# ohinder/OnePhase.jl

Measured on AMD Instinct MI355X. Metric: KKT factor+solve/sec (fp64) at n+m~1e5, nnz~2e6, higher is better.
Workload: dtype f64

## Files before the change

onephase.jl_amd/csrc/asan_driver.cpp:

```cpp
#include <cstdio>
#include <cstdlib>
#include <random>
#include <set>
#include <vector>

#include "numeric.h"
#include "pivots.h"
#include "symbolic.h"

using namespace okkt;

static void csc_lower(int n, const std::set<std::pair<int, int>>& e, std::vector<int64_t>& cp, std::vector<int64_t>& ri) {
  std::vector<std::vector<int>> cols(n);
  for (auto& p : e) cols[std::min(p.first, p.second)].push_back(std::max(p.first, p.second));
  cp.assign(n + 1, 0); ri.clear();
  for (int j = 0; j < n; ++j) { ri.push_back(j); for (int r : cols[j]) if (r != j) ri.push_back(r); cp[j + 1] = (int64_t)ri.size(); }
}

static int run(const char* name, int n, const std::set<std::pair<int, int>>& e, int ordering) {
  std::vector<int64_t> cp, ri;
  csc_lower(n, e, cp, ri);
  SymbolicOptions o;
  o.ordering = ordering;
  Symbolic S;
  const std::string err = analyze_pattern(n, cp.data(), ri.data(), 0, o, nullptr, S);
  if (!err.empty()) { fprintf(stderr, "%s (ordering %d): %s\n", name, ordering, err.c_str()); return 1; }
  std::vector<DfFront> fronts;
  for (int s = 0; s < (int)S.sn_col0.size() - 1 && fronts.size() < 3; ++s) {
    const int k = S.sn_col0[s + 1] - S.sn_col0[s], f = (int)(S.row_ptr[s + 1] - S.row_ptr[s]);
    if (f > 128) fronts.push_back({s, f, k});
  }
  size_t ntask = 0;
  if (!fronts.empty()) {
    std::vector<DfTask> q;
    double model = 0;
    df_build_queue(fronts, 64, 4, 1, true, true, q, &model, true);
    ntask = q.size();
    df_build_queue(fronts, 96, 2, 2, false, false, q, &model, false);
  }
  std::vector<int64_t> fpos(S.nsuper + 1, 0);
  for (int s = 0; s < S.nsuper; ++s)
    fpos[s + 1] = fpos[s] + (S.row_ptr[s + 1] - S.row_ptr[s]) * (int64_t)(S.sn_col0[s + 1] - S.sn_col0[s]);
  for (int skip : {-1, S.nsuper - 1}) {
    PvPlan P;
    const std::string pe = pivot_build_items(S, fpos, 128, skip, P);
    if (!pe.empty()) { fprintf(stderr, "%s (ordering %d): %s\n", name, ordering, pe.c_str()); return 1; }
    std::vector<int> seen(n, 0), next_row(n, -1);
    int64_t entries = 0;
    bool ok = true;
    for (const PvSmall& q : P.small) {
      ok = ok && q.f <= 128 && q.k <= q.f && q.L >= 0 && q.L + (int64_t)q.f * q.k <= fpos[S.nsuper];
      for (int lc = 0; lc < q.k; ++lc) { ++seen[q.col0 + lc]; entries += q.f - lc - 1; }
    }
    std::vector<int> part_owner(P.nparts, -1);
    for (const PvBig& q : P.big) {
      const int s = S.col2sn[q.out], f = (int)(S.row_ptr[s + 1] - S.row_ptr[s]), lc = q.out - S.sn_col0[s];
      ok = ok && f > 128 && q.col == fpos[s] + (int64_t)lc * f && q.rows == S.row_ptr[s] && q.r0 <= q.r1 && q.r1 <= f && q.r1 - q.r0 <= kPvChunkRows;
      ok = ok && q.r0 == (next_row[q.out] < 0 ? lc + 1 : next_row[q.out]);
      next_row[q.out] = q.r1;
      entries += q.r1 - q.r0;
      if (q.part < 0) ++seen[q.out];
      else { ok = ok && q.part < P.nparts && part_owner[q.part] < 0; if (ok) part_owner[q.part] = q.out; }
    }
    for (const PvMerge& q : P.merge) {
      ++seen[q.out];
      ok = ok && q.nparts > 1 && q.part0 >= 0 && q.part0 + q.nparts <= P.nparts;
      for (int c = 0; ok && c < q.nparts; ++c) ok = part_owner[q.part0 + c] == q.out;
    }
    const int ncov = skip < 0 ? n : S.sn_col0[skip];
    for (int c = 0; c < n; ++c) {
      ok = ok && seen[c] == (c < ncov ? 1 : 0);
      if (c < ncov && next_row[c] >= 0) { const int s = S.col2sn[c]; ok = ok && next_row[c] == (int)(S.row_ptr[s + 1] - S.row_ptr[s]); }
    }
    ok = ok && entries == P.entries && P.ncols == ncov;
    if (!ok) { fprintf(stderr, "%s (ordering %d): the pivot-report items do not tile the factor (skip %d)\n", name, ordering, skip); return 1; }
  }
  printf("%-12s ordering %d: n %d nnz(L) %lld supernodes %zu, %zu dataflow tasks\n", name, ordering, n, (long long)S.nnzL, S.sn_col0.size() - 1, ntask);
  return 0;
}

int main() {
  int bad = 0;
  std::mt19937 rng(5);
  {
    const int n = 3000;
    std::set<std::pair<int, int>> e;
    for (int i = 0; i < n; ++i) for (int d = 1; d <= 3; ++d) if (i + d < n) e.insert({i, i + d});
    for (int i = 0; i < n; i += 2) e.insert({i, n - 1});
    for (int o : {0, 3, 4}) bad += run("banded", n, e, o);
  }
  {
    const int g = 14, n = g * g * g;
    std::set<std::pair<int, int>> e;
    auto id = [&](int x, int y, int z) { return (x * g + y) * g + z; };
    for (int x = 0; x < g; ++x) for (int y = 0; y < g; ++y) for (int z = 0; z < g; ++z) {
      if (x + 1 < g) e.insert({id(x, y, z), id(x + 1, y, z)});
      if (y + 1 < g) e.insert({id(x, y, z), id(x, y + 1, z)});
      if (z + 1 < g) e.insert({id(x, y, z), id(x, y, z + 1)});
    }
    for (int o : {0, 3, 4, 5}) bad += run("grid", n, e, o);
  }
  {
    const int n = 12000;
    std::set<std::pair<int, int>> e;
    for (int i = 0; i < n; ++i) for (int d = 1; d <= 12; d += 3) if (i + d < n) e.insert({i, i + d});
    for (int t = 0; t < n / 4; ++t) { const int a = (int)(rng() % n), b = (int)(rng() % n); if (a != b) e.insert({a, b}); }
    for (int o : {0, 5}) bad += run("small-world", n, e, o);
  }
  {
    const int n = 24000;
    std::set<std::pair<int, int>> e;
    for (int i = 0; i < n; ++i) for (int d = 1; d <= 12; d += 3) if (i + d < n) e.insert({i, i + d});
    for (int t = 0; t < n / 4; ++t) { const int a = (int)(rng() % n), b = (int)(rng() % n); if (a != b) e.insert({a, b}); }
    bad += run("small-world-24k", n, e, 5);
  }
  {
    const int n = 600;
    std::set<std::pair<int, int>> e;
    for (int i = 0; i + 1 < n; ++i) { e.insert({i, n - 1}); e.insert({i, i + 1}); }
    for (int o : {0, 1, 3}) bad += run("arrow", n, e, o);
  }
  {
    const int n = 2300;
    std::set<std::pair<int, int>> e;
    for (int i = 1; i < n; ++i) e.insert({0, i});
    bad += run("full-column", n, e, 1);
  }
  if (bad) { fprintf(stderr, "%d case(s) failed\n", bad); return 1; }
  printf("asan driver: all cases clean\n");
  return 0;
}
```

onephase.jl_amd/csrc/numeric.h:

```cpp
#pragma once
#include <hip/hip_runtime.h>

#include <cstdint>
#include <string>
#include <vector>

#include "symbolic.h"

namespace okkt {

struct EaRec { int64_t src; int64_t rel; int rc; int jj; int64_t cut; };
static_assert(sizeof(EaRec) == 32, "two 16-byte loads per record");

struct DevPlan {
  int n = 0, nsuper = 0;
  int has_dup = 0;
  int* sn_col0 = nullptr;
  int64_t* row_ptr = nullptr;
  int* rows = nullptr;
  int64_t* front_pos = nullptr;
  int64_t* cb_shift = nullptr;
  int64_t* child_ptr = nullptr;
  int* children = nullptr;
  int64_t* rel_ptr = nullptr;
  int* rel = nullptr;
  int64_t* cv_pos = nullptr;
  int64_t* aent_ptr = nullptr;
  int64_t* aent_src = nullptr;
  int64_t* aent_dst = nullptr;
  int* perm = nullptr;
  int* sched = nullptr;
  int* task_lo = nullptr;
  int* unit_parent = nullptr;
  double* arena = nullptr;
  const double* vals = nullptr;
  double* dvals = nullptr;
  double* diagadd = nullptr;
  double* xwork = nullptr;
  double* zwork = nullptr;
  double* cv = nullptr;
  double* wbuf = nullptr;
  int64_t* wbuf_pos = nullptr;
  int64_t* bigcol_base = nullptr;
  int64_t* ea_ptr = nullptr;
  int* ea_child = nullptr;
  int* ea_jj = nullptr;
  int64_t* ea_pos = nullptr;
  int* ea_rc = nullptr;
  int64_t* ea_src = nullptr;
  int64_t* ea_rel = nullptr;
  int64_t* ea_cut = nullptr;
  const struct EaRec* ea_rec = nullptr;
  int* cutv = nullptr;
  int64_t* acol_lo = nullptr;
  double* xinv = nullptr;
  double* xtmp = nullptr;
  int64_t* xinv_pos = nullptr;
  double* ypart = nullptr;
  int64_t* ypart_pos = nullptr;
  int solve_mid = 0;
  double* ythin = nullptr;
  int64_t* ythin_pos = nullptr;
  int* ssched = nullptr;
  unsigned long long* sver = nullptr;
  int64_t* sver_pos = nullptr;
  int64_t xw_stride = 0, cv_stride = 0;
  double* invl = nullptr;
  int64_t* invl_pos = nullptr;
  int* sn_owner = nullptr;
  int* col_owner = nullptr;
  int* top_cols = nullptr;
  int* bnd = nullptr;
  int64_t* bnd_cb = nullptr;
  int64_t* bnd_cv = nullptr;
  unsigned long long* counters = nullptr;
  long long want_pos = -1, want_neg = -1;
  double* zero_page = nullptr;
  int df_early_pub = 1;
  int* df_state = nullptr;
  int64_t* df_state_pos = nullptr;
};

enum { kDfD = 0, kDfT = 1, kDfU = 2, kDfTU = 3, kDfTA = 4, kDfTL = 5 };
struct DfTask { int front; int type_nq; int ij; int q0; };
struct DfFront { int s, f, k; };
void df_build_queue(const std::vector<DfFront>& fronts, int workers, int group, int rows_per_task, bool fuse_d, bool split_tu, std::vector<DfTask>& out, double* model_us,
                    bool fuse_tl = false, bool multi_rows = true);
// ... 78 lines not shown
  int flow_levels = 0, flow_off = 0, flow_cnt = 0, flow_maxf = 0, flow_maxk = 0;
  int* flow_flags = nullptr;
  int flow_epoch = 0;
  int dataflow = 1;
  int df_group = 4;
  int df_fuse_d = 1;
  int df_split_tu = 1;
  std::vector<int64_t> front_pos_host;
  int64_t arena_doubles = 0;
  int64_t cb_region_doubles = 0;
  int release_cb = 1;
  int df_fuse_tl = 1;
  int df_rows = 1;
  int df_workers = 256;
  DfTask* df_tasks = nullptr;
  int* df_heads = nullptr;
  int n_df_heads = 0;
  int64_t df_state_ints = 0;
  int diag2 = 1;
  int lookahead = 1;
  int sb_tail_rows = 4000;
  int la_min_tiles = 600;
  std::vector<hipEvent_t> la_events;
  size_t la_used = 0;
  double* vals_owned = nullptr;
  int64_t nnz_in = 0;
  bool profile = false;
  std::vector<hipEvent_t> prof_events;
  size_t prof_used = 0;
  std::vector<double> prof_flops;
  std::vector<std::pair<int, int>> big_fk;
  std::vector<int> sched_host;
  std::vector<int> sn_f, sn_k;
  int schur_sn = -1;
  int64_t schur_gcb = 0;
  int* schur_list = nullptr;
};

std::string numeric_setup(const Symbolic& S, const SymbolicOptions& opts, hipStream_t stream, Numeric& N);
void numeric_release(Numeric& N);

std::string numeric_factor_enqueue(Numeric& N, const double* d_vals, double tol, int which = 0, bool reset_counters = true);
std::string solve_fwd_enqueue(Numeric& N, int which, int R);
std::string solve_bwd_enqueue(Numeric& N, int which, int R);
std::string solve_setup(const Symbolic& S, Numeric& N);
std::string solve_invert_enqueue(Numeric& N, hipStream_t st, const SolveLevel& L, int b_lo, int b_hi);
void solve_permute_in(const Numeric& N, const double* d_rhs, int64_t stride, int nr, int R, const double* d_scale = nullptr);
void solve_permute_out(const Numeric& N, double* d_sol, int64_t stride, int nr, int R, bool accumulate, const double* d_scale = nullptr);
std::string numeric_dist_pack(Numeric& N, int what, int unpack, double* d_buf);
std::string numeric_dist_x(Numeric& N, int mode, double* d_buf);
void numeric_sum_counts_device(Numeric& N, long long* d_out4);
std::string schur_condense_enqueue(Numeric& N, double* d_r2, int nr, int R);
std::string schur_expand_enqueue(Numeric& N, const double* d_x2, int nr, int R);
std::string schur_gather_enqueue(Numeric& N, double* d_r2, int nr, int R);
std::string schur_put_enqueue(Numeric& N, const double* d_x2, int nr, int R);
void schur_export_enqueue(Numeric& N, double* d_S, int64_t ld);
std::string numeric_solve_enqueue(Numeric& N, int R);
void launch_set_shift(const Numeric& N, double delta, int64_t nshift);
std::string df_setup(Numeric& N);
const char* df_build_flags();
std::string df_launch(Numeric& N, const DevPlan& P, const Segment& g, hipStream_t st, double tol);

}
```

onephase.jl_amd/csrc/numeric.hip:

```cpp
#include "numeric.h"
#include "front_device.h"
#include <map>

#include <algorithm>
#include <cmath>
#include <cstdio>
#include <cstdlib>

namespace okkt {


#define OKKT_HIP_TRY(expr)                                                         \
  do {                                                                             \
    hipError_t e__ = (expr);                                                       \
    if (e__ != hipSuccess)                                                         \
      return std::string(#expr) + ": " + hipGetErrorString(e__);                   \
  } while (0)

__global__ void k_fold_counts(DevPlan P) {
  const int c = threadIdx.x;
  if (c >= 4) return;
  unsigned long long sum = 0;
  for (int q = 1; q < kCountSlots; ++q) {
    unsigned long long* w = P.counters + (size_t)q * kCountStride + c;
// ... 305 lines not shown
    }
    int d[NB4];
    double v[NB4];
#pragma unroll
    for (int u = 0; u < NB4; ++u) {
      const int ii = min(lo[u] + lane, rc[u] - 1);
      d[u] = P.rel[rel[u] + ii] - r0;
      v[u] = P.arena[src[u] + ii];
    }
#pragma unroll
    for (int u = 0; u < NB4; ++u) {
      if (q + u < q1) {
        if (lo[u] + lane < hi[u]) base[d[u]] += v[u];
        const int* rl = P.rel + rel[u];
        const double* Ccol = P.arena + src[u];
        int ii = lo[u] + 64 + lane;
        for (; ii + 64 * (kAsmUnroll - 1) < hi[u]; ii += 64 * kAsmUnroll) {
          int dd[kAsmUnroll];
          double vv[kAsmUnroll], oo[kAsmUnroll];
#pragma unroll
          for (int w = 0; w < kAsmUnroll; ++w) dd[w] = rl[ii + 64 * w] - r0;
#pragma unroll
          for (int w = 0; w < kAsmUnroll; ++w) { vv[w] = Ccol[ii + 64 * w]; oo[w] = base[dd[w]]; }
#pragma unroll
          for (int w = 0; w < kAsmUnroll; ++w) base[dd[w]] = oo[w] + vv[w];
        }
        for (; ii < hi[u]; ii += 64) base[rl[ii] - r0] += Ccol[ii];
        __threadfence_block();
      }
    }
  }
  double* col = P.arena + P.front_pos[s] + (size_t)pc * f + r0 + cb_off(P, s, pc, k);
  for (int i = lane; i < n; i += 64) col[i] = base[i];
}






__global__ __launch_bounds__(256) void k_big_diag(DevPlan P, const int* __restrict__ list, int step, int NB, double tol, int dbg_stop) {
  extern __shared__ __attribute__((aligned(16))) double sm[];
  const int tid = threadIdx.x, lane = tid & 63;
  const int wave = __builtin_amdgcn_readfirstlane(tid >> 6);
  const int l15 = lane & 15, l4 = lane >> 4;
  const int s = list[blockIdx.x];
  if (stop_requested_wg(P)) return;
  const int col0 = P.sn_col0[s];
  const int k = P.sn_col0[s + 1] - col0;
  const int f = (int)(P.row_ptr[s + 1] - P.row_ptr[s]);
  const int j0 = step * NB;
  if (j0 >= k) return;
  const int nb = min(NB, k - j0);
  double* Praw = sm;
  double* Lp = Praw + kMW * kPLD;
  double* Wp = Lp + kMW * kPLD;
  double* Ld = Wp + kMW * kPLD;
  double* Xs = Ld + 4 * 32 * kXld;
  double* F = P.arena + P.front_pos[s];

  int ti_s[9], tj_s[9];
#pragma unroll
  for (int q = 0; q < 9; ++q) {
    const int t = 4 * q + wave;
    const int tj = (t >= 8) + (t >= 15) + (t >= 21) + (t >= 26) + (t >= 30) + (t >= 33) + (t >= 35);
    const int start = tj * 8 - tj * (tj - 1) / 2;
// ... 665 lines not shown
        }
      }
      if (wlevel > 0) { wregion[wlevel_seq & 1] = std::max(wregion[wlevel_seq & 1], wlevel); ++wlevel_seq; }
    }
  };
  build(N.levels, parted ? N.part_id : 0);
  if (parted && N.part_id == 0) build(N.levels_top, -1); else N.levels_top.clear();
  if (!(e = upload(N, sched, &d.sched)).empty()) return e;
  if (!(e = upload(N, task_lo, &d.task_lo)).empty()) return e;
  N.flow_levels = N.flow_off = N.flow_cnt = N.flow_maxf = N.flow_maxk = 0;
  if (N.flow && (!parted || parted_tasks)) {
    int nl = 0;
    while (nl < (int)N.levels.size() && N.levels[nl].seg[3].cnt == 0) ++nl;
    if (nl >= 2) {
      N.flow_levels = nl;
      N.flow_off = N.levels[0].seg[0].off;
      for (int l = 0; l < nl; ++l)
        for (int c = 0; c < 3; ++c) { N.flow_cnt += N.levels[l].seg[c].cnt; if (N.levels[l].seg[c].cnt) { N.flow_maxf = std::max(N.flow_maxf, N.levels[l].seg[c].maxf); N.flow_maxk = std::max(N.flow_maxk, N.levels[l].seg[c].maxk); } }
      if (N.flow_cnt == 0) N.flow_levels = 0;
    }
  }
  {
    std::vector<int> unit_parent(ns, -1);
    for (int s2 = 0; s2 < ns; ++s2) {
      if (unit_root[s2] != s2 || S.sn_parent[s2] < 0) continue;
      const int up = unit_root[S.sn_parent[s2]];
      if (up == N.schur_sn) continue;
      if (ulevel[up] < N.flow_levels && (!parted || S.sn_owner[up] == S.sn_owner[s2])) unit_parent[s2] = up;
    }
    if (!(e = upload(N, unit_parent, &d.unit_parent)).empty()) return e;
  }
  if (getenv("OKKT_DEBUG_FRONTS")) fprintf(stderr, "okkt: %d levels of units (%d levels of fronts), %lld tasks of small fronts, longest %d\n", nulev, S.nlevels, (long long)N.n_tasks, N.max_task_len);
  N.release_cb = getenv("OKKT_RELEASE_CB") ? atoi(getenv("OKKT_RELEASE_CB")) : 1;
  if (parted) N.release_cb = 0;
  std::vector<int64_t> fpos(ns + 1, 0), cbshift(ns, 0);
  if (!N.release_cb) {
    for (int s2 = 0; s2 <= ns; ++s2) fpos[s2] = S.front_pos[s2];
    N.arena_doubles = S.arena_doubles;
    N.cb_region_doubles = 0;
  } else {
    for (int s2 = 0; s2 < ns; ++s2) {
      const int64_t f = S.row_ptr[s2 + 1] - S.row_ptr[s2], k = S.sn_col0[s2 + 1] - S.sn_col0[s2];
      fpos[s2 + 1] = fpos[s2] + ((f * k + 1) & ~(int64_t)1);
    }
    const int64_t panels = fpos[ns];
    auto epoch_of = [&](int s2) { const int l = ulevel[unit_root[s2]]; return l < N.flow_levels ? 0 : l - std::max(N.flow_levels, 1) + 1; };
    const int nep = std::max(1, nulev - std::max(N.flow_levels, 1) + 1) + 1;
    std::vector<std::vector<int>> born(nep), dies(nep);
    for (int s2 = 0; s2 < ns; ++s2) {
      const int64_t f = S.row_ptr[s2 + 1] - S.row_ptr[s2], k = S.sn_col0[s2 + 1] - S.sn_col0[s2];
      if (f == k) continue;
      const int p2 = S.sn_parent[s2];
      born[epoch_of(s2)].push_back(s2);
      dies[p2 >= 0 && p2 != N.schur_sn ? epoch_of(p2) : nep - 1].push_back(s2);
    }
    std::map<int64_t, int64_t> freeb;
    int64_t top = 0;
    std::vector<int64_t> cbo(ns, -1), cbsz(ns, 0);
    auto release = [&](int64_t off, int64_t sz) {
      auto it = freeb.emplace(off, sz).first;
      auto nx = std::next(it);
      if (nx != freeb.end() && it->first + it->second == nx->first) { it->second += nx->second; freeb.erase(nx); }
      if (it != freeb.begin()) { auto pv = std::prev(it); if (pv->first + pv->second == it->first) { pv->second += it->second; freeb.erase(it); it = pv; } }
      if (it->first + it->second == top) { top = it->first; freeb.erase(it); }
    };
    for (int ep = 0; ep < nep; ++ep) {
// ... 115 lines not shown
      for (int64_t q = S.rel_ptr[c]; q < S.rel_ptr[c + 1]; ++q) {
        const int64_t slot = fill[bigcol_base[p] + S.rel[q]]++;
        ea_child[slot] = c;
        ea_jj[slot] = (int)(q - S.rel_ptr[c]);
        ea_pos[slot] = S.cv_pos[c] + (q - S.rel_ptr[c]);
        {
          const int64_t kc = S.sn_col0[c + 1] - S.sn_col0[c], fc = S.row_ptr[c + 1] - S.row_ptr[c];
          ea_rc[slot] = (int)(fc - kc);
          ea_rel[slot] = S.rel_ptr[c];
          ea_cut[slot] = cut_pos[c];
          ea_src[slot] = fpos[c] + cbshift[c] + (kc + ea_jj[slot]) * fc + kc;
        }
      }
    }
    if (!(e = upload(N, bigcol_base, &d.bigcol_base)).empty()) return e;
    if (!(e = upload(N, invl_pos, &d.invl_pos)).empty()) return e;
    if (!(e = upload(N, ea_ptr, &d.ea_ptr)).empty()) return e;
    if (!(e = upload(N, ea_child, &d.ea_child)).empty()) return e;
    if (!(e = upload(N, ea_jj, &d.ea_jj)).empty()) return e;
    if (!(e = upload(N, ea_pos, &d.ea_pos)).empty()) return e;
    if (!(e = upload(N, ea_rc, &d.ea_rc)).empty()) return e;
    if (!(e = upload(N, ea_src, &d.ea_src)).empty()) return e;
    if (!(e = upload(N, ea_rel, &d.ea_rel)).empty()) return e;
    if (!(e = upload(N, ea_cut, &d.ea_cut)).empty()) return e;
    {
      std::vector<EaRec> recs(ea_src.size());
      for (size_t t = 0; t < recs.size(); ++t) recs[t] = EaRec{ea_src[t], ea_rel[t], ea_rc[t], ea_jj[t], ea_cut[t]};
      EaRec* dr = nullptr;
      if (!(e = upload(N, recs, &dr)).empty()) return e;
      d.ea_rec = dr;
    }
    if (!(e = upload(N, cutv, &d.cutv)).empty()) return e;
    if (!(e = upload(N, acol_lo, &d.acol_lo)).empty()) return e;
    if (N.schur_sn >= 0) {
      N.schur_gcb = bigcol_base[N.schur_sn];
      if (!(e = upload(N, std::vector<int>{N.schur_sn}, &N.schur_list)).empty()) return e;
    }
    if (!(e = dalloc(N, (size_t)invl_total, &d.invl, true)).empty()) return e;
  }
  if (!(e = dalloc(N, (size_t)N.arena_doubles + 512 + (size_t)S.max_front * 2, &d.arena, false)).empty()) return e;
  if (!(e = dalloc(N, (size_t)S.n, &d.dvals, true)).empty()) return e;
  if (!(e = dalloc(N, (size_t)S.n, &d.diagadd, true)).empty()) return e;
  d.xw_stride = S.n;
  d.cv_stride = S.sum_r;
  if (!(e = dalloc(N, (size_t)S.n * kMaxRhs, &d.xwork, true)).empty()) return e;
  if (!(e = dalloc(N, (size_t)S.n * kMaxRhs, &d.zwork, true)).empty()) return e;
  if (!(e = dalloc(N, (size_t)S.sum_r * kMaxRhs, &d.cv, true)).empty()) return e;
  if (!(e = dalloc(N, (size_t)wtotal + 512, &d.wbuf, true)).empty()) return e;
  if (!(e = dalloc(N, (size_t)kCountSlots * kCountStride, &d.counters, true)).empty()) return e;
  if (!(e = dalloc(N, (size_t)512, &d.zero_page, true)).empty()) return e;
  if (!(e = dalloc(N, (size_t)S.nnz_in, &N.vals_owned, false)).empty()) return e;
  {
    double* raw = nullptr;
    if (!(e = dalloc(N, (size_t)ns / 2 + 8, &raw, true)).empty()) return e;
    N.chain_flags = (int*)raw;
    N.chain_epoch = 0;
    raw = nullptr;
    if (!(e = dalloc(N, (size_t)3 * ns / 2 + 8, &raw, true)).empty()) return e;
    N.flow_flags = (int*)raw;
    N.flow_epoch = 0;
  }
  if (!(e = solve_setup(S, N)).empty()) return e;
  if (!(e = df_setup(N)).empty()) return e;
  const int big_lds = 160 * 1024 - 64;
  OKKT_HIP_TRY(hipFuncSetAttribute((const void*)k_front_small<256>, hipFuncAttributeMaxDynamicSharedMemorySize, big_lds));
  OKKT_HIP_TRY(hipFuncSetAttribute((const void*)k_front_small<256, true>, hipFuncAttributeMaxDynamicSharedMemorySize, big_lds));
// ... 64 lines not shown
std::string numeric_factor_enqueue(Numeric& N, const double* d_vals, double tol, int which, bool reset_counters) {
  DevPlan P = N.d;
  P.vals = d_vals;
  hipStream_t st = N.stream;
  {
    const size_t na = reset_counters ? (size_t)kCountSlots * kCountStride * (sizeof(unsigned long long) / sizeof(unsigned)) : 0;
    const size_t nb = (reset_counters && N.solve_counters) ? (size_t)N.d.nsuper : 0;
    const size_t nc = (N.dataflow && P.df_state) ? (size_t)N.df_state_ints + (size_t)N.n_df_heads * kDfHeadStride : 0;
    if (na + nb + nc) {
      const unsigned grid = (unsigned)std::min<size_t>(2048, (na + nb + nc + 1023) / 1024);
      hipLaunchKernelGGL(k_zero_words, dim3(grid), dim3(256), 0, st, (unsigned*)P.counters, na, (unsigned*)N.solve_counters, nb, (unsigned*)P.df_state, nc);
    }
  }
  if (N.early_check && N.early_device && which == 0 && N.levels_top.empty() && reset_counters) { P.want_pos = N.early_n; P.want_neg = N.early_m; }
  N.la_used = 0;
  if (which == 0) {
    for (size_t l = 0; l < N.inv_level_pending.size(); ++l)
      if (N.inv_level_pending[l] && N.inv_level_events[l]) OKKT_HIP_TRY(hipStreamWaitEvent(st, N.inv_level_events[l], 0));
    if (N.inv_wait && N.inv_event) OKKT_HIP_TRY(hipStreamWaitEvent(st, N.inv_event, 0));
  }
  if (which == 0) std::fill(N.inv_level_pending.begin(), N.inv_level_pending.end(), 0);
  if (which == 0) N.inv_wait = false;
  bool inv_on_aux = false;
  N.early_exited = false;
  std::string e;
  {
    const LaneStreams ss{N.stream, N.stream_masked, N.stream_panel, N.stream_aux};
    e = factor_sched(N, P, which == 0 ? N.levels : N.levels_top, which == 0 ? N.slevels : N.slevels_top, ss, tol,
                     which == 0 && N.levels_top.empty(), inv_on_aux);
    if (!e.empty()) return e;
  }
  if (which == 0 && N.schur_sn >= 0) {
    const int f = N.sn_f[N.schur_sn];
    if (f > 2048) hipLaunchKernelGGL(k_big_assemble_chunked, dim3((f + 3) / 4, 1, (f + kAsmChunk - 1) / kAsmChunk), dim3(256), 0, st, P, N.schur_list);
    else {
      const int lcol = std::max(256, (f + 63) / 64 * 64);
      hipLaunchKernelGGL(k_big_assemble<true>, dim3((f + 3) / 4, 1), dim3(256), (size_t)4 * lcol * sizeof(double), st, P, N.schur_list, lcol);
    }
  }
  const bool per_level = which == 0 && N.levels_top.empty() && !N.inv_level_pending.empty();
  if (inv_on_aux && !per_level) {
    if (!N.inv_event) OKKT_HIP_TRY(hipEventCreateWithFlags(&N.inv_event, hipEventDisableTiming));
    OKKT_HIP_TRY(hipEventRecord(N.inv_event, N.inv_stream ? N.inv_stream : N.stream_aux));
    N.inv_wait = true;
  }
  OKKT_HIP_TRY(hipGetLastError());
  return "";
}

static std::string factor_sched(Numeric& N, DevPlan P, const std::vector<LevelSchedule>& levels, const std::vector<SolveLevel>& slevels,
                                const LaneStreams& ss, double tol, bool in_loop_check, bool& inv_on_aux, size_t l_begin, size_t l_end) {
  const hipStream_t cur = ss.main;
  const int NB = N.nb;
  static const int dbg_syrk = getenv("OKKT_DEBUG_SYRK") ? atoi(getenv("OKKT_DEBUG_SYRK")) : 0;
  static const int split_min_rows = getenv("OKKT_SPLIT_MIN_ROWS") ? atoi(getenv("OKKT_SPLIT_MIN_ROWS")) : 5000;
  static const int dbg_stop = getenv("OKKT_DEBUG_DIAG_STOP") ? atoi(getenv("OKKT_DEBUG_DIAG_STOP")) : 0;
  static const int fuse_max_fronts = getenv("OKKT_FUSE_MAX_FRONTS") ? atoi(getenv("OKKT_FUSE_MAX_FRONTS")) : 8;
  for (size_t l = l_begin; l < std::min(l_end, levels.size()); ++l) {
    const LevelSchedule& L = levels[l];
    if (N.early_check && in_loop_check && (int)l == N.early_level) {
      unsigned long long cnt[6] = {0, 0, 0, 0, 0, 0};
      std::string ec = numeric_read_counts(N, cur, cnt);
      if (!ec.empty()) return ec;
      if (cnt[4] != 0 || cnt[3] > 0 || cnt[2] > 0 || cnt[1] > (unsigned long long)N.early_m || cnt[0] > (unsigned long long)N.early_n) {
        N.early_exited = true;
        return "";
      }
// ... 30 lines not shown
        const int rows_after = g.maxf - (stepA + GS) * NB;
        if (rows_after < N.group_one_rows) return 1;
        return (GS > N.group && rows_after < N.group_switch_rows) ? N.group : GS;
      };
      auto next_event = [&](hipEvent_t* ev) -> std::string {
        if (N.la_used >= N.la_events.size())
          for (int q = 0; q < 64; ++q) { hipEvent_t e2; OKKT_HIP_TRY(hipEventCreateWithFlags(&e2, hipEventDisableTiming)); N.la_events.push_back(e2); }
        *ev = N.la_events[N.la_used++];
        return "";
      };
      auto la_at = [&](int stepA, int gs_cur) {
        const int stepB = stepA + gs_cur;
        if (stepB >= nsteps || !N.lookahead || ss.panel == nullptr || ss.masked == nullptr) return false;
        const int remr = g.maxf - (stepB + gs_at(stepB)) * NB;
        const int Trr = remr > 0 ? (remr + 127) / 128 : 0;
        return (int64_t)Trr * (Trr + 1) / 2 * g.cnt >= N.la_min_tiles;
      };
      const bool use_df = N.dataflow && g.df_cnt > 0 && NB == 128 && dbg_syrk == 0 && dbg_stop == 0 && P.df_state != nullptr;
      const bool seg_la = !use_df && la_at(0, gs_at(0));
      hipStream_t st = cur;
      if (seg_la) {
        hipEvent_t evf;
        std::string e = next_event(&evf);
        if (!e.empty()) return e;
        OKKT_HIP_TRY(hipEventRecord(evf, ss.main));
        OKKT_HIP_TRY(hipStreamWaitEvent(ss.masked, evf, 0));
        st = ss.masked;
      }
      {
        static const int lcol_max = getenv("OKKT_ASM_LCOL") ? atoi(getenv("OKKT_ASM_LCOL")) : 2048;
        int lcol = std::min(lcol_max, std::max(256, (g.maxf + 63) / 64 * 64));
        if (lcol_max <= 0) lcol = 0;
        static const int chunked = getenv("OKKT_ASM_CHUNKED") ? atoi(getenv("OKKT_ASM_CHUNKED")) : 1;
        static const int chunk_min = getenv("OKKT_ASM_CHUNK_MIN") ? atoi(getenv("OKKT_ASM_CHUNK_MIN")) : 2048;
        if (g.maxf > chunk_min && chunked) hipLaunchKernelGGL(k_big_assemble_chunked, dim3((g.maxf + 3) / 4, g.cnt, (g.maxf + kAsmChunk - 1) / kAsmChunk), dim3(256), 0, st, P, list);
        else if (g.maxf <= 2048) hipLaunchKernelGGL(k_big_assemble<true>, dim3((g.maxf + 3) / 4, g.cnt), dim3(256), (size_t)4 * lcol * sizeof(double), st, P, list, lcol);
        else hipLaunchKernelGGL(k_big_assemble<false>, dim3((g.maxf + 3) / 4, g.cnt), dim3(256), (size_t)4 * lcol * sizeof(double), st, P, list, lcol);
      }
      auto launch_syrk = [&](hipStream_t sst, int stepA, int npan, int tstep, int head, int par, int cs, int sub = 0) -> std::string {
        const int rem = g.maxf - (head == 1 ? tstep : stepA) * NB;
        if (rem <= 0) return "";
        const int T = (rem + 127) / 128;
        const int Tr = std::max(T - cs, 0);
        int ntile = T * (T + 1) / 2;
        if (head == 1) ntile = sub == 1 ? 1 : (sub == 2 ? T - 1 : T);
        else if (head == 2) { ntile = 0; for (int c = 0; c < cs && c < T; ++c) ntile += T - c; }
        else if (head == 3) ntile = Tr * (Tr + 1) / 2;
        if (ntile == 0) return "";
        static const int small_max = getenv("OKKT_SYRK_SMALL_TILES") ? atoi(getenv("OKKT_SYRK_SMALL_TILES")) : 1500;
        const bool narrow = (head == 0 || head == 3) && dbg_syrk == 0 && (int64_t)ntile * g.cnt <= small_max;
        if (narrow) ntile = head == 0 ? T * (T + 1) : Tr * (Tr + 1);
        if (ntile <= 0) return "";
        const dim3 grid((ntile + 7) / 8 * 8, g.cnt);
        const int wofs = par * GS * NB;
        const bool prof = N.profile && (head == 0 || head == 3);
        if (prof) {
          double fl = 0;
          for (int q = 0; q < g.cnt; ++q) {
            const int s = N.sched_host[g.off + q];
            const int kk = N.sn_k[s], ff = N.sn_f[s];
            const int j0 = stepA * NB;
            if (j0 >= kk) continue;
            if (head == 1 && tstep * NB >= kk) continue;
            const double K = std::min(npan * NB, kk - j0);
            const double t0 = std::min(tstep * NB, kk);
            const double remq = ff - t0;
            const double w2 = std::min<double>(cs * 128, remq);
            const double remr = remq - w2;
// ... 271 lines not shown
```

Baseline: 56.15.

## Add staged big-front assembly kernel driven by precomputed per-chunk piece records

Precomputes on the host, per big front column and row chunk, a list of contiguous child contribution-block pieces and the range of original-matrix entries. A new kernel walks these pieces with double-buffered register loads and accumulates into an LDS column before writing it out with aligned double2 stores. It becomes the default for all big-front groups and the Schur front, replacing the older search-based chunked and whole-column assembly kernels. This is meant to cut per-item lookup and irregular-access cost during extend-add. In exchange it adds host preprocessing, device memory for the records, and launches chunked grids even for small fronts.

```diff
diff --git a/onephase.jl_amd/csrc/asan_driver.cpp b/onephase.jl_amd/csrc/asan_driver.cpp
--- a/onephase.jl_amd/csrc/asan_driver.cpp
+++ b/onephase.jl_amd/csrc/asan_driver.cpp
@@ -4,6 +4,7 @@
 #include <set>
 #include <vector>
 
+#include "asm_pieces.h"
 #include "numeric.h"
 #include "pivots.h"
 #include "symbolic.h"
@@ -15,6 +16,85 @@
   for (auto& p : e) cols[std::min(p.first, p.second)].push_back(std::max(p.first, p.second));
   cp.assign(n + 1, 0); ri.clear();
   for (int j = 0; j < n; ++j) { ri.push_back(j); for (int r : cols[j]) if (r != j) ri.push_back(r); cp[j + 1] = (int64_t)ri.size(); }
+}
+
+static bool check_asm_pieces(const Symbolic& S, int chunk) {
+  const int ns = S.nsuper;
+  std::vector<char> big(ns, 0);
+  std::vector<int64_t> cb_base(ns, 0);
+  int64_t top = 0;
+  for (int s = 0; s < ns; ++s) {
+    const int64_t f = S.row_ptr[s + 1] - S.row_ptr[s], k = S.sn_col0[s + 1] - S.sn_col0[s];
+    big[s] = f > 128;
+    cb_base[s] = top + k * f + k;
+    top += f * f + (s & 1);
+  }
+  AsmPlan A;
+  if (!asm_build_pieces(S, big, cb_base, chunk, A).empty()) return false;
+  std::vector<std::vector<int>> kids(ns);
+  for (int c = 0; c < ns; ++c) if (S.sn_parent[c] >= 0) kids[S.sn_parent[c]].push_back(c);
+  int64_t items = 0, pieces = 0;
+  for (int p = 0; p < ns; ++p) {
+    if (!big[p]) { if (A.unit_base[p] != -1) return false; continue; }
+    const int64_t f = S.row_ptr[p + 1] - S.row_ptr[p];
+    const int nchunks = (int)((f + chunk - 1) / chunk);
+    for (int64_t pc = 0; pc < f; ++pc) {
+      std::vector<int> ic, ijj, done;
+      for (int c : kids[p]) {
+        const int* rb = S.rel.data() + S.rel_ptr[c];
+        const int* re = S.rel.data() + S.rel_ptr[c + 1];
+        const int* it = std::lower_bound(rb, re, (int)pc);
+        if (it != re && *it == pc) { ic.push_back(c); ijj.push_back((int)(it - rb)); }
+      }
+      done = ijj;
+      items += (int64_t)ic.size();
+      int64_t a_next = -1;
+      for (int t = 0; t < nchunks; ++t) {
+        const AsmUnit& U = A.units[(size_t)(A.unit_base[p] + (int64_t)t * f + pc)];
+        const int64_t r0 = std::max<int64_t>(pc, (int64_t)t * chunk), r1 = std::min<int64_t>(f, (int64_t)(t + 1) * chunk);
+        if (r0 >= r1) { if (U.np != 0 || U.na != 0) return false; continue; }
+        if (U.np < 0 || U.piece0 < 0 || U.piece0 + U.np > (int64_t)A.pieces.size()) return false;
+        if (U.na < 0 || U.a0 < S.aent_ptr[p] || U.a0 + U.na > S.aent_ptr[p + 1]) return false;
+        for (int64_t e = U.a0; e < U.a0 + U.na; ++e) if (S.aent_dst[e] < pc * f + r0 || S.aent_dst[e] >= pc * f + r1) return false;
+        if (a_next >= 0 && U.a0 != a_next) return false;
+        a_next = U.a0 + U.na;
+        int q = 0;
+        for (int i = 0; i < U.np; ++i, ++pieces) {
+          const AsmPiece& R = A.pieces[(size_t)(U.piece0 + i)];
+          if (R.n <= 0) return false;
+          for (; q < (int)ic.size(); ++q) {
+            const int c = ic[q];
+            const int rc = (int)(S.rel_ptr[c + 1] - S.rel_ptr[c]);
+            if (done[q] < rc && S.rel[S.rel_ptr[c] + done[q]] < r1) break;
+          }
+          if (q == (int)ic.size()) return false;
+          const int c = ic[q];
+          const int64_t fc = S.row_ptr[c + 1] - S.row_ptr[c];
+          const int rc = (int)(S.rel_ptr[c + 1] - S.rel_ptr[c]);
+          int hi = done[q];
+          while (hi < rc && S.rel[S.rel_ptr[c] + hi] < r1) ++hi;
+          if (S.rel[S.rel_ptr[c] + done[q]] < r0) return false;
+          if (R.src != cb_base[c] + (int64_t)ijj[q] * fc + done[q] || R.rel != S.rel_ptr[c] + done[q] || R.n != hi - done[q]) return false;
+          done[q] = hi;
+          ++q;
+        }
+        for (int j = 0; j < (int)ic.size(); ++j) {
+          const int c = ic[j];
+          const int rc = (int)(S.rel_ptr[c + 1] - S.rel_ptr[c]);
+          if (done[j] < rc && S.rel[S.rel_ptr[c] + done[j]] < r1) return false;
+        }
+      }
+      for (int j = 0; j < (int)ic.size(); ++j) if (done[j] != (int)(S.rel_ptr[ic[j] + 1] - S.rel_ptr[ic[j]])) return false;
+      if (a_next >= 0) {
+        const int64_t* dst = S.aent_dst.data();
+        const int64_t lo = std::lower_bound(dst + S.aent_ptr[p], dst + S.aent_ptr[p + 1], pc * f + pc) - dst;
+        const int64_t hi = std::lower_bound(dst + S.aent_ptr[p], dst + S.aent_ptr[p + 1], (pc + 1) * f) - dst;
+        const AsmUnit& U0 = A.units[(size_t)(A.unit_base[p] + (pc / chunk) * f + pc)];
+        if (U0.a0 != lo || a_next != hi) return false;
+      }
+    }
+  }
+  return items == A.items && pieces == (int64_t)A.pieces.size();
 }
 
 static int run(const char* name, int n, const std::set<std::pair<int, int>>& e, int ordering) {
@@ -75,6 +155,8 @@
     ok = ok && entries == P.entries && P.ncols == ncov;
     if (!ok) { fprintf(stderr, "%s (ordering %d): the pivot-report items do not tile the factor (skip %d)\n", name, ordering, skip); return 1; }
   }
+  for (int chunk : {512, 1024, 48})
+    if (!check_asm_pieces(S, chunk)) { fprintf(stderr, "%s (ordering %d): the assembly pieces do not tile the extend-add items (chunk %d)\n", name, ordering, chunk); return 1; }
   printf("%-12s ordering %d: n %d nnz(L) %lld supernodes %zu, %zu dataflow tasks\n", name, ordering, n, (long long)S.nnzL, S.sn_col0.size() - 1, ntask);
   return 0;
 }
@@ -126,6 +208,17 @@
     for (int i = 1; i < n; ++i) e.insert({0, i});
     bad += run("full-column", n, e, 1);
   }
+  {
+    const int nl = 30, nsep = 2300, n = 3 * nl + nsep;
+    std::set<std::pair<int, int>> e;
+    for (int g = 0; g < 3; ++g) {
+      for (int i = 0; i < nl; ++i) for (int j = i + 1; j < nl; ++j) e.insert({g * nl + i, g * nl + j});
+      for (int i = 0; i < nl; ++i)
+        for (int r = 0; r < nsep; ++r)
+          if (g == 0 || r == 0 || (g == 1 && r % 2 == 1) || (g == 2 && (r % 3 == 2 || (r > 1020 && r < 1030)))) e.insert({g * nl + i, 3 * nl + r});
+    }
+    bad += run("three-chunks", n, e, 1);
+  }
   if (bad) { fprintf(stderr, "%d case(s) failed\n", bad); return 1; }
   printf("asan driver: all cases clean\n");
   return 0;
diff --git a/onephase.jl_amd/csrc/asm_pieces.h b/onephase.jl_amd/csrc/asm_pieces.h
--- /dev/null
+++ b/onephase.jl_amd/csrc/asm_pieces.h
@@ -0,0 +1,106 @@
+#pragma once
+#include <algorithm>
+#include <cstdint>
+#include <string>
+#include <vector>
+
+#include "symbolic.h"
+
+namespace okkt {
+
+struct alignas(16) AsmPiece { int64_t src; int rel; int n; };
+static_assert(sizeof(AsmPiece) == 16, "one 16-byte load per piece and lane");
+struct alignas(32) AsmUnit { int64_t piece0; int64_t a0; int np; int na; int pad[2]; };
+static_assert(sizeof(AsmUnit) == 32, "host and device agree on the record");
+
+struct AsmPlan {
+  std::vector<int64_t> unit_base;
+  std::vector<AsmUnit> units;
+  std::vector<AsmPiece> pieces;
+  int64_t items = 0;
+  int64_t bytes() const { return (int64_t)(unit_base.size() * sizeof(int64_t) + units.size() * sizeof(AsmUnit) + pieces.size() * sizeof(AsmPiece)); }
+};
+
+inline std::string asm_build_pieces(const Symbolic& S, const std::vector<char>& big, const std::vector<int64_t>& cb_base, int chunk, AsmPlan& A) {
+  A = AsmPlan();
+  const int ns = S.nsuper;
+  if ((int)big.size() < ns || (int)cb_base.size() < ns || chunk <= 0) return "assembly records: the inputs do not cover the supernodes";
+  if (S.rel.size() > (size_t)INT32_MAX) return "assembly records: the rel lists pass 2^31 entries";
+  A.unit_base.assign(ns, -1);
+  std::vector<int64_t> col_base(ns, -1);
+  int64_t ncols = 0, nunits = 0;
+  for (int s = 0; s < ns; ++s)
+    if (big[s]) {
+      const int64_t f = S.row_ptr[s + 1] - S.row_ptr[s];
+      if (f > INT32_MAX) return "assembly records: a front's order is out of range";
+      col_base[s] = ncols;
+      ncols += f;
+      A.unit_base[s] = nunits;
+      nunits += f * ((f + chunk - 1) / chunk);
+    }
+  std::vector<int64_t> iptr(ncols + 1, 0);
+  for (int c = 0; c < ns; ++c) {
+    const int p = S.sn_parent[c];
+    if (p < 0 || !big[p]) continue;
+    for (int64_t q = S.rel_ptr[c]; q < S.rel_ptr[c + 1]; ++q) ++iptr[col_base[p] + S.rel[q] + 1];
+  }
+  for (int64_t i = 0; i < ncols; ++i) iptr[i + 1] += iptr[i];
+  A.items = iptr[ncols];
+  std::vector<int> ichild(A.items), ijj(A.items);
+  {
+    std::vector<int64_t> fill(iptr.begin(), iptr.end() - 1);
+    for (int c = 0; c < ns; ++c) {
+      const int p = S.sn_parent[c];
+      if (p < 0 || !big[p]) continue;
+      for (int64_t q = S.rel_ptr[c]; q < S.rel_ptr[c + 1]; ++q) {
+        const int64_t slot = fill[col_base[p] + S.rel[q]]++;
+        ichild[slot] = c;
+        ijj[slot] = (int)(q - S.rel_ptr[c]);
+      }
+    }
+  }
+  std::vector<int64_t> cut_pos(ns, -1);
+  std::vector<int> cutv;
+  for (int c = 0; c < ns; ++c) {
+    const int p = S.sn_parent[c];
+    if (p < 0 || !big[p]) continue;
+    const int64_t fp = S.row_ptr[p + 1] - S.row_ptr[p];
+    const int* rb = S.rel.data() + S.rel_ptr[c];
+    const int* re = S.rel.data() + S.rel_ptr[c + 1];
+    cut_pos[c] = (int64_t)cutv.size();
+    const int nchunks = (int)((fp + chunk - 1) / chunk);
+    for (int t = 0; t <= nchunks; ++t) cutv.push_back((int)(std::lower_bound(rb, re, (int)std::min<int64_t>((int64_t)t * chunk, INT32_MAX)) - rb));
+  }
+  A.units.assign((size_t)nunits, AsmUnit{0, 0, 0, 0, {0, 0}});
+  for (int s = 0; s < ns; ++s) {
+    if (!big[s]) continue;
+    const int64_t f = S.row_ptr[s + 1] - S.row_ptr[s];
+    const int nchunks = (int)((f + chunk - 1) / chunk);
+    const int64_t e0 = S.aent_ptr[s], e1 = S.aent_ptr[s + 1];
+    const int64_t* dst = S.aent_dst.data();
+    for (int t = 0; t < nchunks; ++t)
+      for (int64_t pc = 0; pc < f; ++pc) {
+        AsmUnit& U = A.units[(size_t)(A.unit_base[s] + (int64_t)t * f + pc)];
+        U.piece0 = (int64_t)A.pieces.size();
+        const int64_t r0 = std::max<int64_t>(pc, (int64_t)t * chunk), r1 = std::min<int64_t>(f, (int64_t)(t + 1) * chunk);
+        if (r0 >= r1) continue;
+        const int64_t a0 = std::lower_bound(dst + e0, dst + e1, pc * f + r0) - dst;
+        const int64_t a1 = std::lower_bound(dst + a0, dst + e1, pc * f + r1) - dst;
+        U.a0 = a0;
+        U.na = (int)(a1 - a0);
+        for (int64_t q = iptr[col_base[s] + pc]; q < iptr[col_base[s] + pc + 1]; ++q) {
+          const int c = ichild[q], jj = ijj[q];
+          const int64_t fc = S.row_ptr[c + 1] - S.row_ptr[c];
+          const int rc = (int)(fc - (S.sn_col0[c + 1] - S.sn_col0[c]));
+          const int* cut = cutv.data() + cut_pos[c];
+          const int lo = std::max(jj, cut[t]), hi = std::min(rc, cut[t + 1]);
+          if (lo >= hi) continue;
+          A.pieces.push_back(AsmPiece{cb_base[c] + (int64_t)jj * fc + lo, (int)(S.rel_ptr[c] + lo), hi - lo});
+        }
+        U.np = (int)((int64_t)A.pieces.size() - U.piece0);
+      }
+  }
+  return "";
+}
+
+}
diff --git a/onephase.jl_amd/csrc/numeric.h b/onephase.jl_amd/csrc/numeric.h
--- a/onephase.jl_amd/csrc/numeric.h
+++ b/onephase.jl_amd/csrc/numeric.h
@@ -5,6 +5,7 @@
 #include <string>
 #include <vector>
 
+#include "asm_pieces.h"
 #include "symbolic.h"
 
 namespace okkt {
@@ -53,6 +54,9 @@
   const struct EaRec* ea_rec = nullptr;
   int* cutv = nullptr;
   int64_t* acol_lo = nullptr;
+  int64_t* asm_unit_base = nullptr;
+  const AsmUnit* asm_unit = nullptr;
+  const AsmPiece* asm_piece = nullptr;
   double* xinv = nullptr;
   double* xtmp = nullptr;
   int64_t* xinv_pos = nullptr;
@@ -197,6 +201,8 @@
   std::vector<std::pair<int, int>> big_fk;
   std::vector<int> sched_host;
   std::vector<int> sn_f, sn_k;
+  int asm_staged = 1;
+  int64_t asm_record_bytes = 0;
   int schur_sn = -1;
   int64_t schur_gcb = 0;
   int* schur_list = nullptr;
diff --git a/onephase.jl_amd/csrc/numeric.hip b/onephase.jl_amd/csrc/numeric.hip
--- a/onephase.jl_amd/csrc/numeric.hip
+++ b/onephase.jl_amd/csrc/numeric.hip
@@ -361,6 +361,111 @@
   }
   double* col = P.arena + P.front_pos[s] + (size_t)pc * f + r0 + cb_off(P, s, pc, k);
   for (int i = lane; i < n; i += 64) col[i] = base[i];
+}
+
+#ifndef OKKT_ASM_STAGE
+#define OKKT_ASM_STAGE 2
+#endif
+#ifndef OKKT_ASM_STAGED_CHUNK
+#define OKKT_ASM_STAGED_CHUNK 512
+#endif
+constexpr int kAsmStage = OKKT_ASM_STAGE;
+constexpr int kAsmStagedChunk = OKKT_ASM_STAGED_CHUNK;
+__global__ __launch_bounds__(256) void k_big_assemble_staged(DevPlan P, const int* __restrict__ list) {
+  __shared__ __attribute__((aligned(16))) double sm[4 * kAsmStagedChunk];
+  const int lane = threadIdx.x & 63, wv = __builtin_amdgcn_readfirstlane((int)(threadIdx.x >> 6));
+  const int s = list[blockIdx.y];
+  if (stop_requested_wave(P)) return;
+  const int col0 = P.sn_col0[s];
+  const int k = P.sn_col0[s + 1] - col0;
+  const int f = (int)(P.row_ptr[s + 1] - P.row_ptr[s]);
+  const int pc = blockIdx.x * 4 + wv;
+  if (pc >= f) return;
+  const int t = blockIdx.z;
+  const int r0 = max(pc, t * kAsmStagedChunk), r1 = min(f, (t + 1) * kAsmStagedChunk);
+  if (r0 >= r1) return;
+  const AsmUnit U = P.asm_unit[P.asm_unit_base[s] + (int64_t)t * f + pc];
+  double* base = sm + wv * kAsmStagedChunk;
+  const int n = r1 - r0;
+  constexpr int D = kAsmStage;
+  int np = 0, p = 0, off = 0, cn = 1;
+  int rsl = 0, rsh = 0, rrel = 0, rn = 0;
+  int64_t csrc = 0, crel = 0;
+  auto seek = [&]() {
+    csrc = (int64_t)(((uint64_t)(uint32_t)__builtin_amdgcn_readlane(rsh, p) << 32) | (uint32_t)__builtin_amdgcn_readlane(rsl, p));
+    crel = __builtin_amdgcn_readlane(rrel, p);
+    cn = __builtin_amdgcn_readlane(rn, p);
+  };
+  auto load_block = [&](int p0) {
+    np = min(64, U.np - p0);
+    const AsmPiece R = P.asm_piece[U.piece0 + p0 + min(lane, np - 1)];
+    rsl = (int)(uint32_t)R.src; rsh = (int)(R.src >> 32); rrel = R.rel; rn = R.n;
+    p = 0; off = 0;
+    seek();
+  };
+  int dA[D], dB[D], cA[D], cB[D];
+  double vA[D], vB[D];
+  auto issue = [&](int (&d)[D], double (&v)[D], int (&c)[D]) {
+#pragma unroll
+    for (int u = 0; u < D; ++u) {
+      const int ii = min(off + lane, cn - 1);
+      d[u] = P.rel[crel + ii];
+      v[u] = P.arena[csrc + ii];
+      c[u] = p < np ? min(64, cn - off) : 0;
+      if (p < np) {
+        off += 64;
+        if (off >= cn) {
+          ++p; off = 0;
+          if (p < np) seek();
+        }
+      }
+    }
+    asm volatile("" ::: "memory");
+  };
+  auto apply = [&](const int (&d)[D], const double (&v)[D], const int (&c)[D]) {
+#pragma unroll
+    for (int u = 0; u < D; ++u) {
+      if (lane < c[u]) base[d[u] - r0] += v[u];
+      asm volatile("" ::: "memory");
+    }
+  };
+  if (U.np > 0) { load_block(0); issue(dA, vA, cA); }
+  for (int i = lane; i < n; i += 64) base[i] = 0.0;
+  __threadfence_block();
+  if (pc < k) {
+    const int64_t lo = U.a0, hi = U.a0 + U.na;
+    const int64_t cbase = (int64_t)pc * f + r0;
+    if (!P.has_dup) {
+      for (int64_t e = lo + lane; e < hi; e += 64) base[(int)(P.aent_dst[e] - cbase)] = P.vals[P.aent_src[e]];
+    } else if (lane == 0) {
+      for (int64_t e = lo; e < hi; ++e) base[(int)(P.aent_dst[e] - cbase)] += P.vals[P.aent_src[e]];
+    }
+    __threadfence_block();
+    if (lane == 0 && pc >= r0 && pc < r1) base[pc - r0] += P.diagadd[col0 + pc];
+    __threadfence_block();
+  }
+  if (U.np > 0)
+    for (int p0 = 0;;) {
+      for (;;) {
+        issue(dB, vB, cB);
+        apply(dA, vA, cA);
+        if (cB[0] == 0) break;
+        issue(dA, vA, cA);
+        apply(dB, vB, cB);
+        if (cA[0] == 0) break;
+      }
+      p0 += 64;
+      if (p0 >= U.np) break;
+      load_block(p0);
+      issue(dA, vA, cA);
+    }
+  __threadfence_block();
+  double* col = P.arena + P.front_pos[s] + (size_t)pc * f + r0 + cb_off(P, s, pc, k);
+  const int head = (int)(((uintptr_t)col >> 3) & 1);
+  if (head && lane == 0) col[0] = base[0];
+  const int n2 = (n - head) >> 1;
+  for (int i = lane; i < n2; i += 64) *(double2*)(col + head + 2 * i) = make_double2(base[head + 2 * i], base[head + 2 * i + 1]);
+  if (((n - head) & 1) && lane == 0) col[n - 1] = base[n - 1];
 }
 
 
@@ -1092,6 +1197,7 @@
   }
   if (getenv("OKKT_DEBUG_FRONTS")) fprintf(stderr, "okkt: %d levels of units (%d levels of fronts), %lld tasks of small fronts, longest %d\n", nulev, S.nlevels, (long long)N.n_tasks, N.max_task_len);
   N.release_cb = getenv("OKKT_RELEASE_CB") ? atoi(getenv("OKKT_RELEASE_CB")) : 1;
+  N.asm_staged = getenv("OKKT_ASM_STAGED") ? atoi(getenv("OKKT_ASM_STAGED")) : 1;
   if (parted) N.release_cb = 0;
   std::vector<int64_t> fpos(ns + 1, 0), cbshift(ns, 0);
   if (!N.release_cb) {
@@ -1273,6 +1379,27 @@
     }
     if (!(e = upload(N, cutv, &d.cutv)).empty()) return e;
     if (!(e = upload(N, acol_lo, &d.acol_lo)).empty()) return e;
+    {
+      std::vector<char> big(ns, 0);
+      std::vector<int64_t> cb_base(ns, 0);
+      for (int s = 0; s < ns; ++s) {
+        const int64_t kc = S.sn_col0[s + 1] - S.sn_col0[s], fc = S.row_ptr[s + 1] - S.row_ptr[s];
+        big[s] = wpos[s] >= 0;
+        cb_base[s] = fpos[s] + cbshift[s] + kc * fc + kc;
+      }
+      AsmPlan A;
+      if (!(e = asm_build_pieces(S, big, cb_base, kAsmStagedChunk, A)).empty()) return e;
+      AsmUnit* du = nullptr;
+      AsmPiece* dp = nullptr;
+      if (!(e = upload(N, A.unit_base, &d.asm_unit_base)).empty()) return e;
+      if (!(e = upload(N, A.units, &du)).empty()) return e;
+      if (!(e = upload(N, A.pieces, &dp)).empty()) return e;
+      d.asm_unit = du;
+      d.asm_piece = dp;
+      N.asm_record_bytes = A.bytes();
+      if (getenv("OKKT_DEBUG_FRONTS")) fprintf(stderr, "okkt: staged assembly records %.1f MB (%lld units, %lld pieces of %lld items) = %.2f %% of the front arena\n", A.bytes() * 1e-6,
+                                              (long long)A.units.size(), (long long)A.pieces.size(), (long long)A.items, 100.0 * A.bytes() / (8.0 * N.arena_doubles));
+    }
     if (N.schur_sn >= 0) {
       N.schur_gcb = bigcol_base[N.schur_sn];
       if (!(e = upload(N, std::vector<int>{N.schur_sn}, &N.schur_list)).empty()) return e;
@@ -1403,7 +1530,9 @@
   }
   if (which == 0 && N.schur_sn >= 0) {
     const int f = N.sn_f[N.schur_sn];
-    if (f > 2048) hipLaunchKernelGGL(k_big_assemble_chunked, dim3((f + 3) / 4, 1, (f + kAsmChunk - 1) / kAsmChunk), dim3(256), 0, st, P, N.schur_list);
+    static const int chunked_on = getenv("OKKT_ASM_CHUNKED") ? atoi(getenv("OKKT_ASM_CHUNKED")) : 1;
+    if (N.asm_staged && chunked_on) hipLaunchKernelGGL(k_big_assemble_staged, dim3((f + 3) / 4, 1, (f + kAsmStagedChunk - 1) / kAsmStagedChunk), dim3(256), 0, st, P, N.schur_list);
+    else if (f > 2048) hipLaunchKernelGGL(k_big_assemble_chunked, dim3((f + 3) / 4, 1, (f + kAsmChunk - 1) / kAsmChunk), dim3(256), 0, st, P, N.schur_list);
     else {
       const int lcol = std::max(256, (f + 63) / 64 * 64);
       hipLaunchKernelGGL(k_big_assemble<true>, dim3((f + 3) / 4, 1), dim3(256), (size_t)4 * lcol * sizeof(double), st, P, N.schur_list, lcol);
@@ -1500,8 +1629,10 @@
         int lcol = std::min(lcol_max, std::max(256, (g.maxf + 63) / 64 * 64));
         if (lcol_max <= 0) lcol = 0;
         static const int chunked = getenv("OKKT_ASM_CHUNKED") ? atoi(getenv("OKKT_ASM_CHUNKED")) : 1;
-        static const int chunk_min = getenv("OKKT_ASM_CHUNK_MIN") ? atoi(getenv("OKKT_ASM_CHUNK_MIN")) : 2048;
-        if (g.maxf > chunk_min && chunked) hipLaunchKernelGGL(k_big_assemble_chunked, dim3((g.maxf + 3) / 4, g.cnt, (g.maxf + kAsmChunk - 1) / kAsmChunk), dim3(256), 0, st, P, list);
+        static const int chunk_min_env = getenv("OKKT_ASM_CHUNK_MIN") ? atoi(getenv("OKKT_ASM_CHUNK_MIN")) : -1;
+        const int chunk_min = chunk_min_env >= 0 ? chunk_min_env : (N.asm_staged ? 0 : 2048);
+        if (g.maxf > chunk_min && chunked && N.asm_staged) hipLaunchKernelGGL(k_big_assemble_staged, dim3((g.maxf + 3) / 4, g.cnt, (g.maxf + kAsmStagedChunk - 1) / kAsmStagedChunk), dim3(256), 0, st, P, list);
+        else if (g.maxf > chunk_min && chunked) hipLaunchKernelGGL(k_big_assemble_chunked, dim3((g.maxf + 3) / 4, g.cnt, (g.maxf + kAsmChunk - 1) / kAsmChunk), dim3(256), 0, st, P, list);
         else if (g.maxf <= 2048) hipLaunchKernelGGL(k_big_assemble<true>, dim3((g.maxf + 3) / 4, g.cnt), dim3(256), (size_t)4 * lcol * sizeof(double), st, P, list, lcol);
         else hipLaunchKernelGGL(k_big_assemble<false>, dim3((g.maxf + 3) / 4, g.cnt), dim3(256), (size_t)4 * lcol * sizeof(double), st, P, list, lcol);
       }
```

New measurement: 57.92, median of 6. 3.2% higher.
